# ethz-asl/okvis

Measured on NVIDIA B200. Metric: keyframe-window optimize() iters/sec (10KF/2k-lm stereo), higher is better.
Workload: dtype f64

## Files before the change

okvis_b200/csrc/okb_estimator.cu:

```cuda
#include <cuda_runtime.h>

#include <algorithm>
#include <cstddef>
#include <cstdio>
#include <cstdlib>
#include <cstring>
#include <string>
#include <thread>
#include <vector>

#include "okb_ctx.h"
#include "okb_hostpack.hpp"
#include "okb_graph.cuh"
#include "okb_kernels.cuh"
#include "okb_marg.cuh"

using namespace okb;

static std::string g_create_error;

#define OKB_CUDA(ctx, call)                                                                             \
  do {                                                                                                  \
    cudaError_t e_ = (call);                                                                            \
    if (e_ != cudaSuccess) {                                                                            \
// ... 361 lines not shown
    if (marg_n > kMaxMarg || marg_nb > kMaxMargBlocks) { c->set_error("marginalisation prior too large"); return OKB_ERR_CAPACITY; }
    int col = 0;
    for (int b = 0; b < marg_nb; ++b) {
      const int kind = D->marg->block_kind[b];
      const uint32_t idx = D->marg->block_idx[b];
      const int lim = kind == OKB_BLOCK_POSE ? K : kind == OKB_BLOCK_SPEED_BIAS ? NSB : kind == OKB_BLOCK_EXTRINSICS ? NE : -1;
      if (lim < 0) { c->set_error("marginalisation prior: unknown block kind"); return OKB_ERR_INVALID_ARG; }
      if ((int)idx >= lim) { c->set_error("marginalisation prior: block index out of range"); return OKB_ERR_INVALID_ARG; }
      if (kind != OKB_BLOCK_EXTRINSICS) col += (kind == OKB_BLOCK_SPEED_BIAS) ? 9 : 6;
      marg_xdim += (kind == OKB_BLOCK_SPEED_BIAS) ? 9 : 7;
    }
    if (col != marg_n) { c->set_error("marginalisation prior dimension mismatch"); return OKB_ERR_INVALID_ARG; }
  }
  for (int i = 0; i < D->n_pose_priors; ++i)
    if ((int)D->pose_priors[i].pose_idx >= K) { c->set_error("pose prior index out of range"); return OKB_ERR_INVALID_ARG; }
  for (int i = 0; i < D->n_sb_priors; ++i)
    if ((int)D->sb_priors[i].sb_idx >= NSB) { c->set_error("speed/bias prior index out of range"); return OKB_ERR_INVALID_ARG; }
  for (int t = 0; t < D->n_imu_terms; ++t) {
    const okb_imu_term& T = D->imu_terms[t];
    if ((int)T.pose0 >= K || (int)T.pose1 >= K || (int)T.sb0 >= NSB || (int)T.sb1 >= NSB ||
        (uint64_t)T.sample_offset + (uint64_t)T.sample_count > (uint64_t)D->n_imu_samples || T.sample_count < 2) {
      c->set_error("IMU term index out of range");
      return OKB_ERR_INVALID_ARG;
    }
  }
  for (int i = 0; i < D->n_obs; ++i) {
    const okb_observation& ob = D->obs[i];
    if ((int)ob.pose_idx >= K || (int)ob.lm_idx >= L || (int)ob.ext_idx >= NE || (int)ob.cam_idx >= NC) {
      c->set_error("observation index out of range");
      return OKB_ERR_INVALID_ARG;
    }
    if (!(ob.sqrt_info > 0.0)) { c->set_error("observation with non-positive sqrt information"); return OKB_ERR_INVALID_ARG; }
  }
  if (smemA2_bytes(K, 4 * ((6 * K + 1 + 3) / 4), 0) > (size_t)c->smem_optin) { c->set_error("window does not fit kernel A shared memory"); return OKB_ERR_CAPACITY; }

  WinStore& S = c->wins[win];
  S.uploaded = false;
  WinCaps need{K, L, D->n_obs, D->n_imu_samples, D->n_imu_terms, NE, NC, std::max(D->n_pose_priors, D->n_sb_priors), marg_n};
  need = caps_max(need, S.reserve);
  need.T = std::max(need.T, need.K);
  if (!S.arena || !caps_cover(S.caps, need)) {
    if (S.done_idx >= 0) OKB_CUDA(c, cudaEventSynchronize(c->done_ring[S.done_idx]));
    int rc = plan_arena(c, win, S.arena ? caps_max(S.caps, need) : need);
    if (rc) return rc;
  }
  S.cmd_used = 0;
  int rc = cmd_reserve(c, S, full_upload_bytes(need));
  if (rc) return rc;
  unsigned char* q;
  q = cmd_put(S, CMD_RESET_GRAPH, 0, (uint32_t)NE, (uint32_t)NC, 8 * 7 * (size_t)NE + sizeof(okb_camera) * NC);
  std::memcpy(q, D->extrinsics, 8 * 7 * (size_t)NE);
  std::memcpy(q + 8 * 7 * (size_t)NE, D->cameras, sizeof(okb_camera) * NC);
  q = cmd_put(S, CMD_SET_FRAMES, 0, (uint32_t)K, (uint32_t)NSB, 8 * (7 * (size_t)K + 9 * (size_t)NSB));
  std::memcpy(q, D->poses, 8 * 7 * (size_t)K);
  if (NSB) std::memcpy(q + 8 * 7 * (size_t)K, D->speed_bias, 8 * 9 * (size_t)NSB);
  q = cmd_put(S, CMD_SET_LANDMARKS, (uint32_t)L, 0, 1, 8 * 4 * (size_t)L);
  std::memcpy(q, D->landmarks, 8 * 4 * (size_t)L);
  if (D->n_obs) {
    q = cmd_put(S, CMD_ADD_OBS, (uint32_t)D->n_obs, 0, 0, sizeof(okb_observation) * (size_t)D->n_obs);
    std::memcpy(q, D->obs, sizeof(okb_observation) * (size_t)D->n_obs);
  }
  q = cmd_put(S, CMD_SET_IMU, 0, (uint32_t)D->n_imu_terms, (uint32_t)D->n_imu_samples,
              sizeof(okb_imu_term) * D->n_imu_terms + sizeof(okb_imu_sample) * (size_t)D->n_imu_samples);
  if (D->n_imu_terms) std::memcpy(q, D->imu_terms, sizeof(okb_imu_term) * D->n_imu_terms);
  if (D->n_imu_samples) std::memcpy(q + sizeof(okb_imu_term) * D->n_imu_terms, D->imu_samples, sizeof(okb_imu_sample) * (size_t)D->n_imu_samples);
  q = cmd_put(S, CMD_SET_POSE_PRIORS, (uint32_t)D->n_pose_priors, 0, 0, sizeof(okb_pose_prior) * D->n_pose_priors);
  if (D->n_pose_priors) std::memcpy(q, D->pose_priors, sizeof(okb_pose_prior) * D->n_pose_priors);
// ... 52 lines not shown
    std::vector<std::thread> th;
    th.reserve(T);
    for (int t = 0; t < T; ++t)
      th.emplace_back([=, &rcs]() {
        for (int i = t; i < count; i += T) {
          const int rc = upload_pack(c, first + i, descs + i);
          if (rc) { rcs[t] = rc; return; }
        }
      });
    for (auto& x : th) x.join();
  }
  for (int t = 0; t < T; ++t)
    if (rcs[t]) return rcs[t];
  return commit_range(c, first, count);
}

static int delta_begin(okb_ctx* c, int win, size_t extra, WinStore** S, WinDev** W) {
  if (!c || win < 0 || win >= c->max_windows) return OKB_ERR_INVALID_ARG;
  if (!c->wins[win].uploaded) { c->set_error("window slot not uploaded"); return OKB_ERR_INVALID_ARG; }
  cudaSetDevice(c->device);
  *S = &c->wins[win];
  *W = &c->host[win];
  return cmd_reserve(c, **S, extra + sizeof(CmdHeader) + 64);
}

extern "C" int okb_window_add_frame(okb_ctx* c, int win, const double* pose, const double* speed_bias, const okb_imu_term* term,
                                    const okb_imu_sample* samples, int n_samples) {
  WinStore* S; WinDev* W;
  if (!pose || (term && (!samples || n_samples < 2))) return OKB_ERR_INVALID_ARG;
  int rc = delta_begin(c, win, 16 * 8 + sizeof(okb_imu_term) + sizeof(okb_imu_sample) * (size_t)std::max(n_samples, 0) + sizeof(CmdHeader), &S, &W);
  if (rc) return rc;
  const int K1 = W->K + 1, NSB1 = W->NSB + (speed_bias ? 1 : 0);
  if (K1 > S->caps.K || NSB1 > S->caps.K || 6 * K1 + 9 * NSB1 > kMaxDense) { c->set_error("okb_window_add_frame: frame capacity exceeded (okb_window_reserve)"); return OKB_ERR_CAPACITY; }
  if (smemA2_bytes(K1, 4 * ((6 * K1 + 1 + 3) / 4), 0) > (size_t)c->smem_optin) { c->set_error("window does not fit kernel A shared memory"); return OKB_ERR_CAPACITY; }
  if (term) {
    if ((int)term->pose0 >= K1 || (int)term->pose1 >= K1 || (int)term->sb0 >= NSB1 || (int)term->sb1 >= NSB1 ||
        (uint64_t)term->sample_offset + term->sample_count > (uint64_t)n_samples || term->sample_count < 2) {
      c->set_error("IMU term index out of range");
      return OKB_ERR_INVALID_ARG;
    }
    if (W->n_imu + 1 > S->caps.T || W->n_samples + n_samples > S->caps.S) { c->set_error("okb_window_add_frame: IMU capacity exceeded (okb_window_reserve)"); return OKB_ERR_CAPACITY; }
  }
  if (c->shard_world > 1 && shard_box_doubles(K1, 4 * ((6 * K1 + 1 + 3) / 4)) > (size_t)c->shard_box_cap) { c->set_error("window exceeds the shard mailbox"); return OKB_ERR_CAPACITY; }
  unsigned char* q = cmd_put(*S, CMD_ADD_FRAME, 0, 0, speed_bias ? 1u : 0u, 8 * 16);
  std::memcpy(q, pose, 56);
  if (speed_bias) std::memcpy(q + 56, speed_bias, 72); else std::memset(q + 56, 0, 72);
  W->K = K1; W->NSB = NSB1;
  if (term) {
    q = cmd_put(*S, CMD_ADD_IMU_TERM, (uint32_t)n_samples, 0, 0, sizeof(okb_imu_term) + sizeof(okb_imu_sample) * (size_t)n_samples);
    std::memcpy(q, term, sizeof(okb_imu_term));
    std::memcpy(q + sizeof(okb_imu_term), samples, sizeof(okb_imu_sample) * (size_t)n_samples);
    okb_imu_term mirror = *term;
    mirror.sample_offset += (uint32_t)W->n_samples;
    S->terms.push_back(mirror);
    W->n_imu += 1; W->n_samples += n_samples;
  }
  derive_dims(*W);
  return OKB_OK;
}

extern "C" int okb_window_remove_frame(okb_ctx* c, int win, uint32_t pose_idx, uint32_t sb_idx) {
  WinStore* S; WinDev* W;
  int rc = delta_begin(c, win, 0, &S, &W);
  if (rc) return rc;
  const bool has_sb = sb_idx != 0xffffffffu;
  if ((int)pose_idx >= W->K || (has_sb && (int)sb_idx >= W->NSB) || W->K < 2) { c->set_error("okb_window_remove_frame: index out of range"); return OKB_ERR_INVALID_ARG; }
  cmd_put(*S, CMD_REMOVE_FRAME, 0, pose_idx, sb_idx, 0);
// ... 435 lines not shown

extern "C" int64_t okb_window_h2d_bytes(const okb_ctx* c, int win) {
  if (!c || win < 0 || win >= c->max_windows || !c->wins[win].uploaded) return 0;
  return (int64_t)(c->wins[win].h2d_bytes + sizeof(WinDev));
}

extern "C" int okb_window_reset(okb_ctx* c, int first, int count) {
  int rc = check_range(c, first, count);
  if (rc) return rc;
  cudaSetDevice(c->device);
  for (int i = first; i < first + count; ++i) {
    const WinStore& S = c->wins[i];
    const WinDev& W = c->host[i];
    if (W.K != S.K_init || W.NSB != S.NSB_init || W.L != S.L_init) { c->set_error("okb_window_reset: the window changed shape since its last full upload"); return OKB_ERR_INVALID_ARG; }
  }
  rc = commit_range(c, first, count);
  if (rc) return rc;
  cudaStream_t xs = c->stream_xfer;
  bool waited[okb_ctx::kDoneRing] = {};
  for (int i = first; i < first + count; ++i) {
    const WinStore& S = c->wins[i];
    if (S.done_idx >= 0 && !waited[S.done_idx]) {
      OKB_CUDA(c, cudaStreamWaitEvent(xs, c->done_ring[S.done_idx], 0));
      waited[S.done_idx] = true;
    }
  }
  k_reset<<<count, 128, 0, xs>>>(c->d_wins, first, 1);
  c->launches += 1;
  OKB_CUDA(c, cudaGetLastError());
  return OKB_OK;
}

struct RoundPlan {
  int max_chunks = 1, max_imu = 0, max_cx = 1, max_K = 1, acc_copies = 1, chol_smem = 1, solve_threads = S_THREADS, gxQ = 1, shard = 0, push_gx = 1;
  size_t smA = 0, smS = 0, smQ = 0;
};
static int plan_rounds(okb_ctx* c, int first, int count, RoundPlan& P) {
  P = RoundPlan();
  int chol_smem = 1;
  int acc_copies = 1;
  const size_t sm_two = ((size_t)c->smem_per_sm - 2048) / 2;
  for (int i = first; i < first + count; ++i)
    if (smemA2_bytes(c->host[i].K, c->host[i].dcp, 1) > std::min((size_t)c->smem_optin, sm_two) &&
        smemA2_bytes(c->host[i].K, c->host[i].dcp, 0) <= sm_two) acc_copies = 0;
  for (int i = first; i < first + count; ++i)
    if (smemA2_bytes(c->host[i].K, c->host[i].dcp, acc_copies) > (size_t)c->smem_optin) acc_copies = 0;
  int maxL = 1;
  for (int i = first; i < first + count; ++i) {
    const WinDev& W = c->host[i];
    P.max_chunks = std::max(P.max_chunks, W.n_chunks);
    P.max_imu = std::max(P.max_imu, W.n_imu);
    P.smA = std::max(P.smA, smemA2_bytes(W.K, W.dcp, acc_copies));
    P.max_cx = std::max(P.max_cx, (W.L + L1_THREADS - 1) / L1_THREADS);
    P.max_K = std::max(P.max_K, W.K);
    {
      const int wm = smemS_bytes(W.d, W.dc, W.K, W.marg_n, W.n_imu, 1) <= (size_t)c->smem_optin ? 1
                   : smemS_bytes(W.d, W.dc, W.K, W.marg_n, W.n_imu, 2) <= (size_t)c->smem_optin ? 2 : 0;
      if (wm == 0 || chol_smem == 0) chol_smem = 0;
      else if (wm == 2) chol_smem = 2;
    }
    P.smQ = std::max(P.smQ, (size_t)W.NS * sizeof(SlotCtx));
    maxL = std::max(maxL, W.L);
  }
  for (int i = first; i < first + count; ++i) {
    const WinDev& W = c->host[i];
    P.smS = std::max(P.smS, smemS_bytes(W.d, W.dc, W.K, W.marg_n, W.n_imu, chol_smem));
  }
  if (P.smS > (size_t)c->smem_optin) { c->set_error("window does not fit kernel S shared memory"); return OKB_ERR_CAPACITY; }
  if (const char* force = getenv("OKB_SOLVE_MODE")) {
    const int m = atoi(force);
    if ((m == 0 || m == 2) && chol_smem != 0 && !(chol_smem == 2 && m == 2)) {
      chol_smem = m;
      P.smS = 0;
      for (int i = first; i < first + count; ++i) {
        const WinDev& W = c->host[i];
        P.smS = std::max(P.smS, smemS_bytes(W.d, W.dc, W.K, W.marg_n, W.n_imu, chol_smem));
      }
      if (P.smS > (size_t)c->smem_optin) { c->set_error("window does not fit kernel S shared memory"); return OKB_ERR_CAPACITY; }
    }
  }
  P.acc_copies = acc_copies; P.chol_smem = chol_smem;
  P.solve_threads = (2 * count <= c->sm_count) ? 512 : S_THREADS;
  P.gxQ = std::max(1, std::min((maxL + 127) / 128, (4 * c->sm_count + count - 1) / count));
  P.shard = c->shard_world > 1 ? 1 : 0;
  P.push_gx = std::max(1, std::min(16, c->sm_count / std::max(1, count)));
  return OKB_OK;
}

static int launch_rounds(okb_ctx* c, int first, int count, const okb_solve_options& opt, int rounds, const RoundPlan& P) {
  for (int r = 0; r < rounds; ++r) {
    const dim3 gridA(P.max_chunks, count);
    static const bool imu_serial = getenv("OKB_IMU_SERIAL") != nullptr;
    if (P.max_imu > 0 && imu_serial) {
      k_imu<<<dim3((P.max_imu + 32 / IMU_G - 1) / (32 / IMU_G), count), 32, smemI_bytes(), c->stream>>>(c->d_wins, first);
      c->launches += 1;
    } else if (P.max_imu > 0) {
      cudaEventRecord(c->ev_round, c->stream);
      cudaStreamWaitEvent(c->stream_imu, c->ev_round, 0);
      k_imu<<<dim3((P.max_imu + 32 / IMU_G - 1) / (32 / IMU_G), count), 32, smemI_bytes(), c->stream_imu>>>(c->d_wins, first);
      cudaEventRecord(c->ev_imu, c->stream_imu);
      c->launches += 1;
    }
    prof_begin(c, 0);
    k_linearize<<<dim3(P.max_cx, P.max_K, count), L1_THREADS, 0, c->stream>>>(c->d_wins, first);
    k_lmblock<<<dim3(P.max_cx, count), 128, 0, c->stream>>>(c->d_wins, first);
    k_schur<<<gridA, A2_THREADS, P.smA, c->stream>>>(c->d_wins, first, P.acc_copies, opt.max_iterations);
    if (P.shard) {
      k_shard_push<<<dim3(P.push_gx, count), 256, 0, c->stream>>>(c->d_wins, first);
      c->launches += 1;
    } else if (P.max_chunks > 1) { k_reduce_partials<<<dim3(8, count), 256, 0, c->stream>>>(c->d_wins, first); c->launches += 1; }
    prof_end(c);
    c->launches += 3;
    if (P.max_imu > 0 && !imu_serial) cudaStreamWaitEvent(c->stream, c->ev_imu, 0);
    prof_begin(c, 1);
    if (P.solve_threads == 512) k_solve<512><<<count, 512, P.smS, c->stream>>>(c->d_wins, first, opt, P.chol_smem);
    else k_solve<S_THREADS><<<count, S_THREADS, P.smS, c->stream>>>(c->d_wins, first, opt, P.chol_smem);
    prof_end(c);
    c->launches += 1;
  }
  OKB_CUDA(c, cudaGetLastError());
  return OKB_OK;
}

static int launch_quality(okb_ctx* c, int first, int count, const RoundPlan& P) {
  prof_begin(c, 2);
  k_quality<<<dim3(P.gxQ, count), 128, P.smQ, c->stream>>>(c->d_wins, first);
  prof_end(c);
  c->launches += 1;
  OKB_CUDA(c, cudaGetLastError());
  return OKB_OK;
}

static int run_rounds(okb_ctx* c, int first, int count, const okb_solve_options& opt, int rounds, bool with_quality) {
  RoundPlan P;
  int rc = plan_rounds(c, first, count, P);
  if (rc) return rc;
  static const bool no_graph = getenv("OKB_NO_GRAPH") != nullptr;
  if (c->profile || no_graph || c->shard_world > 1) {
    rc = launch_rounds(c, first, count, opt, rounds, P);
// ... 488 lines not shown
```

okvis_b200/csrc/okb_kernels_lm.cuh:

```cuda
#pragma once
#include "okb_estimator.cuh"

namespace okb {

constexpr int L1_THREADS = 128;
constexpr int A2_THREADS = 192;
constexpr int A2_TILE = 32;
constexpr int kPartH = 32;

struct SlotCtx {
  SlotXf xf;
  CamIntr cam;
  int frame;
  int valid;
};
static_assert(sizeof(SlotCtx) % 8 == 0, "SlotCtx is copied as doubles");

__device__ inline void build_slot_ctx(const WinDev& W, int tid, int nthr) {
  for (int s = tid; s < W.NS; s += nthr) {
    const SlotInfo si = W.slots[s];
    SlotCtx sc;
    sc.valid = si.valid; sc.frame = s / W.CP;
    if (si.valid) { make_slot_xf(W.pose_c + 7 * si.pose_idx, W.ext + 7 * si.ext_idx, sc.xf); cam_load(W.cams[si.cam_idx], sc.cam); }
    else { for (int k = 0; k < 9; ++k) sc.xf.R[k] = 0; for (int k = 0; k < 3; ++k) sc.xf.t[k] = 0; cam_load(W.cams[0], sc.cam); }
    W.slot_ctx[s] = sc;
  }
}

__global__ void __launch_bounds__(L1_THREADS) k_linearize(const WinDev* __restrict__ wins, int win_first) {
  const WinDev& W = wins[win_first + blockIdx.z];
  const SolverState* st = W.st;
  if (st->done) return;
  const int f = blockIdx.y;
  const int cx = blockIdx.x;
  if (f >= W.K || cx * L1_THREADS >= W.L) return;
  const int tid = threadIdx.x;
  const int L = W.L, CP = W.CP;

  __shared__ SlotCtx slots[32];
// ... 162 lines not shown
  for (int c = 0; c < 3; ++c) {
    const double s2 = sc3[c] * sc3[c];
    E[c] = fmin(fmax(s2 * hd[c], kMinDiag), kMaxDiag) / s2;
  }
  const double R[6] = {H[0] + mu * E[0], H[1], H[2], H[3] + mu * E[1], H[4], H[5] + mu * E[2]};
  double Lc[6], Li[6];
  if (chol3(R, Lc)) linv3(Lc, Li);
  else {
#pragma unroll
    for (int i = 0; i < 6; ++i) Li[i] = 0.0;
    st->numeric_fail = 1;
  }
  double* Ro = W.lm_Rinv + 6 * (size_t)l;
  Ro[0] = Li[0] * Li[0] + Li[1] * Li[1] + Li[3] * Li[3];
  Ro[1] = Li[1] * Li[2] + Li[3] * Li[4];
  Ro[2] = Li[3] * Li[5];
  Ro[3] = Li[2] * Li[2] + Li[4] * Li[4];
  Ro[4] = Li[4] * Li[5];
  Ro[5] = Li[5] * Li[5];
  double* gs = W.lm_g[cur ^ 1] + 3 * (size_t)l;
  double* Es = W.lm_E[cur ^ 1] + 3 * (size_t)l;
#pragma unroll
  for (int c = 0; c < 3; ++c) { gs[c] = gl[c]; Es[c] = E[c]; }
  double* Lo = W.lm_Li + 9 * (size_t)l;
#pragma unroll
  for (int i = 0; i < 6; ++i) Lo[i] = Li[i];
  Lo[6] = Li[0] * gl[0];
  Lo[7] = Li[1] * gl[0] + Li[2] * gl[1];
  Lo[8] = Li[3] * gl[0] + Li[4] * gl[1] + Li[5] * gl[2];
}

constexpr int kLiStride = 9;

__host__ __device__ inline int schur_ldy(int dcp) { return dcp + 2; }

__host__ __device__ inline size_t schur_acc_doubles(int K) { return (size_t)(6 * K + 1) * (6 * K + 2) / 2; }
__host__ __device__ inline size_t smemA2_bytes(int K, int dcp, int acc_copies) {
  size_t b = 16;
  b += ((size_t)3 * A2_TILE * schur_ldy(dcp) + 8) * sizeof(double);
  b += (size_t)2 * K * 6 * A2_TILE * sizeof(double);
  b += (size_t)2 * A2_TILE * kLiStride * sizeof(double);
  b += (size_t)2 * A2_TILE * 4 * sizeof(double);
  b += (size_t)K * 4 * sizeof(double);
  b += (size_t)acc_copies * schur_acc_doubles(K) * sizeof(double);
  return b;
}

__device__ __forceinline__ uint32_t smem_u32(const void* p) { return (uint32_t)__cvta_generic_to_shared(p); }
__device__ __forceinline__ void mbar_init(uint64_t* bar, uint32_t count) {
  asm volatile("mbarrier.init.shared::cta.b64 [%0], %1;" ::"r"(smem_u32(bar)), "r"(count) : "memory");
}
__device__ __forceinline__ void mbar_arrive_expect_tx(uint64_t* bar, uint32_t bytes) {
  asm volatile("mbarrier.arrive.expect_tx.shared::cta.b64 _, [%0], %1;" ::"r"(smem_u32(bar)), "r"(bytes) : "memory");
}
__device__ __forceinline__ void bulk_g2s(void* dst, const void* src, uint32_t bytes, uint64_t* bar) {
  asm volatile("cp.async.bulk.shared::cluster.global.mbarrier::complete_tx::bytes [%0], [%1], %2, [%3];" ::"r"(smem_u32(dst)), "l"(src),
               "r"(bytes), "r"(smem_u32(bar))
               : "memory");
}
__device__ __forceinline__ void mbar_wait(uint64_t* bar, uint32_t parity) {
  uint32_t ok;
  do {
    asm volatile("{\n\t.reg .pred p;\n\tmbarrier.try_wait.parity.shared::cta.b64 p, [%1], %2;\n\tselp.u32 %0, 1, 0, p;\n\t}"
                 : "=r"(ok)
                 : "r"(smem_u32(bar)), "r"(parity)
                 : "memory");
  } while (!ok);
}
__device__ __forceinline__ void fence_proxy_async() { asm volatile("fence.proxy.async.shared::cta;" ::: "memory"); }

__global__ void __launch_bounds__(A2_THREADS, 2) k_schur(const WinDev* __restrict__ wins, int win_first, int acc_copies, int max_iterations) {
  const WinDev& W = wins[win_first + blockIdx.y];
  SolverState* st = W.st;
  if (st->done) return;
  if (st->iteration >= max_iterations) return;
  const int chunk = blockIdx.x;
  if (chunk >= W.n_chunks) return;
  const int tid = threadIdx.x;
  const int K = W.K, dc = W.dc, dcp = W.dcp, L = W.L;
  const int ldy = schur_ldy(dcp);

  extern __shared__ __align__(16) unsigned char smem_raw[];
  uint64_t* mbar = reinterpret_cast<uint64_t*>(smem_raw);
  double* Yt = reinterpret_cast<double*>(smem_raw + 16);
  double* sMb = Yt + (size_t)3 * A2_TILE * ldy + 8;
  double* sLib = sMb + (size_t)2 * K * 6 * A2_TILE;
  double* sXb = sLib + 2 * A2_TILE * kLiStride;
  double* tws = sXb + 2 * A2_TILE * 4;
  double* Sp = W.partA + (size_t)chunk * W.partA_stride;
  const bool acc_smem = acc_copies > 0;
  const int acc_n = (dc + 1) * (dc + 2) / 2;
  double* Sacc = acc_smem ? tws + 4 * K : Sp;
  const int n_acc = acc_smem ? acc_copies * acc_n : dcp * dcp;

  for (int f = tid; f < K; f += A2_THREADS) {
    tws[4 * f] = W.pose_c[7 * f]; tws[4 * f + 1] = W.pose_c[7 * f + 1]; tws[4 * f + 2] = W.pose_c[7 * f + 2];
  }
  for (int i = tid; i < n_acc; i += A2_THREADS) Sacc[i] = 0.0;

  const int lm_begin = chunk * W.lm_per_chunk;
  const int lm_end = min(L, lm_begin + W.lm_per_chunk);

  const int warp = tid >> 5, lane = tid & 31;
  if (tid == 0) { mbar_init(&mbar[0], 1); mbar_init(&mbar[1], 1); fence_proxy_async(); }
  __syncthreads();
  uint32_t phase_bits = 0;
  auto stage = [&](int base, int buf, uint32_t tr) {
    const int fa = tr & 0xffu, fb = tr >> 8;
    if (fa > fb || warp != A2_THREADS / 32 - 1) return;
    double* sM = sMb + (size_t)buf * K * 6 * A2_TILE;
    double* sLi = sLib + buf * A2_TILE * kLiStride;
    double* sX = sXb + buf * A2_TILE * 4;
    if (lane == 0) {
      const uint32_t m_bytes = (uint32_t)(fb - fa + 1) * 6 * A2_TILE * 8;
      mbar_arrive_expect_tx(&mbar[buf], m_bytes + A2_TILE * kLiStride * 8 + A2_TILE * 4 * 8);
      bulk_g2s(sM + (size_t)fa * 6 * A2_TILE, W.lm_M + lm_M_index(base, fa, K), m_bytes, &mbar[buf]);
      bulk_g2s(sLi, W.lm_Li + (size_t)kLiStride * base, A2_TILE * kLiStride * 8, &mbar[buf]);
      bulk_g2s(sX, W.lm_c + 4 * (size_t)base, A2_TILE * 4 * 8, &mbar[buf]);
    }
  };

  int cur_fa = -1, cur_fb = -1, lane_fmax = 0;
  int KS = 1, kg = 0, n_act = 0, n_pairs = 0, n_pass = 1;
  int a_off = 0, b_off = 0, row0 = 0, col0 = 0;
  bool on = false, aug = false;
  double acc[36];
#pragma unroll
  for (int i = 0; i < 36; ++i) acc[i] = 0.0;

  auto decode = [&](int item, int fa) {
    aug = false;
    on = item < n_act;
    if (!on) return;
    if (item < n_pairs) {
      int i = (int)((sqrtf(8.0f * (float)item + 1.0f) - 1.0f) * 0.5f);
      while (i * (i + 1) / 2 > item) --i;
      while ((i + 1) * (i + 2) / 2 <= item) ++i;
      const int j = item - i * (i + 1) / 2;
      row0 = 6 * (fa + i); col0 = 6 * (fa + j);
      lane_fmax = fa + i;
    } else {
      aug = true;
      row0 = dc; col0 = 6 * (fa + item - n_pairs);
      lane_fmax = fa + item - n_pairs;
    }
    a_off = row0; b_off = col0;
  };
  double* Ssm = tws + 4 * K;
  auto flush_smem = [&](int copy) {
    double* cp = Ssm + (size_t)copy * acc_n + col0;
    if (aug) {
      double* rp = cp + (size_t)dc * (dc + 1) / 2;
#pragma unroll
      for (int c = 0; c < 6; ++c) rp[c] += acc[c];
    } else if (row0 == col0) {
#pragma unroll
      for (int r = 0; r < 6; ++r) {
        double* rp = cp + (size_t)(row0 + r) * (row0 + r + 1) / 2;
#pragma unroll
        for (int c = 0; c <= r; ++c) rp[c] += acc[r * 6 + c];
      }
    } else {
#pragma unroll
      for (int r = 0; r < 6; ++r) {
        double* rp = cp + (size_t)(row0 + r) * (row0 + r + 1) / 2;
        double t[6];
#pragma unroll
        for (int c = 0; c < 6; ++c) t[c] = rp[c];
#pragma unroll
        for (int c = 0; c < 6; ++c) rp[c] = t[c] + acc[r * 6 + c];
      }
    }
  };
  auto flush_global = [&]() {
#pragma unroll
    for (int i = 0; i < 36; ++i) {
      const int rr = row0 + i / 6, cc = col0 + i % 6;
      if ((!aug || i < 6) && cc <= rr) Sp[(size_t)rr * dcp + cc] += acc[i];
    }
  };
  auto flush = [&]() {
    for (int o = KS >> 1; o > 0; o >>= 1) {
#pragma unroll
      for (int i = 0; i < 36; ++i) acc[i] += __shfl_down_sync(0xffffffffu, acc[i], o);
    }
    if (on && kg == 0) { if (acc_smem) flush_smem(0); else flush_global(); }
#pragma unroll
    for (int i = 0; i < 36; ++i) acc[i] = 0.0;
  };

#ifdef OKB_SCHUR_PROF
  const bool prof = (tid == 0 && chunk == 0);
  unsigned long long t_ph = 0, ph[8] = {0, 0, 0, 0, 0, 0, 0, 0};
  auto now = []() { return (unsigned long long)clock64(); };
#define SCHUR_MARK(i) do { if (prof) { const unsigned long long n_ = now(); ph[i] += n_ - t_ph; t_ph = n_; } } while (0)
  if (prof) t_ph = now();
#else
#define SCHUR_MARK(i) do { } while (0)
#endif
  int buf = 0;
  const int last_tile = (lm_end - 1) >> 5;
  uint32_t tr_cur = (lm_begin < lm_end) ? W.tile_range[lm_begin >> 5] : 1u;
  uint32_t tr_n1 = (lm_begin + A2_TILE < lm_end) ? W.tile_range[(lm_begin >> 5) + 1] : 1u;
  if (lm_begin < lm_end) stage(lm_begin, 0, tr_cur);
  for (int base = lm_begin; base < lm_end; base += A2_TILE) {
    const uint32_t tr_n2 = W.tile_range[min((base >> 5) + 2, last_tile)];
    const int nl = min(A2_TILE, lm_end - base);
    const double* sM = sMb + (size_t)buf * K * 6 * A2_TILE;
    const double* sLi = sLib + buf * A2_TILE * kLiStride;
    const double* sX = sXb + buf * A2_TILE * 4;
    if ((tr_cur & 0xffu) <= (tr_cur >> 8)) {
      mbar_wait(&mbar[buf], (phase_bits >> buf) & 1u);
      phase_bits ^= 1u << buf;
    }
    __syncthreads();
    SCHUR_MARK(0);
    if (base + A2_TILE < lm_end) stage(base + A2_TILE, buf ^ 1, tr_n1);
    SCHUR_MARK(6);
    const uint32_t tr = tr_cur;
    tr_cur = tr_n1; tr_n1 = tr_n2;
    const int fa = tr & 0xffu, fb = tr >> 8;
    buf ^= 1;
    if (fa > fb) continue;
    const int u = fb - fa + 1;
    if (fa != cur_fa || fb != cur_fb) {
      flush();
      cur_fa = fa; cur_fb = fb;
      const int um = fb - fa + 1;
      n_pairs = um * (um + 1) / 2;
      n_act = n_pairs + um;
      constexpr int NW = A2_THREADS / 32;
      const int ipw = (n_act + NW - 1) / NW;
      if (ipw <= 32) {
        n_pass = 1;
        KS = 1;
        while (2 * KS <= 8 && 2 * KS * ipw <= 32) KS *= 2;
        kg = lane % KS;
        const int il = lane / KS;
        decode(warp * ipw + il, fa);
        on = on && il < ipw;
      } else {
        n_pass = (n_act + A2_THREADS - 1) / A2_THREADS;
        KS = 1; kg = 0;
      }
    }
    SCHUR_MARK(1);
    if (tid < A2_TILE) {
      const int ll = tid;
      double* yz = Yt + (size_t)(3 * ll) * ldy + dc;
      const bool v = ll < nl;
      yz[0] = v ? sLi[ll * kLiStride + 6] : 0.0;
      yz[ldy] = v ? sLi[ll * kLiStride + 7] : 0.0;
      yz[2 * ldy] = v ? sLi[ll * kLiStride + 8] : 0.0;
    }
    for (int pidx = tid; pidx < A2_TILE * u; pidx += A2_THREADS) {
      const int ll = pidx % A2_TILE, f = fa + pidx / A2_TILE;
      double* y0 = Yt + (size_t)(3 * ll) * ldy + 6 * f;
      double* y1 = y0 + ldy;
      double* y2 = y1 + ldy;
      double M0 = 0, M1 = 0, M2 = 0, M3 = 0, M4 = 0, M5 = 0;
      if (ll < nl) {
        const double* sp = sM + (size_t)(f * 6) * A2_TILE + ll;
        M0 = sp[0]; M1 = sp[A2_TILE]; M2 = sp[2 * A2_TILE]; M3 = sp[3 * A2_TILE]; M4 = sp[4 * A2_TILE]; M5 = sp[5 * A2_TILE];
      }
      if (M0 != 0.0 || M3 != 0.0 || M5 != 0.0) {
        const double* Li = sLi + ll * kLiStride;
        const double w = sX[ll * 4 + 3];
        const double p0 = sX[ll * 4] - tws[4 * f] * w, p1 = sX[ll * 4 + 1] - tws[4 * f + 1] * w, p2 = sX[ll * 4 + 2] - tws[4 * f + 2] * w;
        const double N00 = M0 * Li[0], N01 = M0 * Li[1] + M1 * Li[2], N02 = M0 * Li[3] + M1 * Li[4] + M2 * Li[5];
        const double N10 = M1 * Li[0], N11 = M1 * Li[1] + M3 * Li[2], N12 = M1 * Li[3] + M3 * Li[4] + M4 * Li[5];
        const double N20 = M2 * Li[0], N21 = M2 * Li[1] + M4 * Li[2], N22 = M2 * Li[3] + M4 * Li[4] + M5 * Li[5];
        y0[0] = -w * N00; y0[1] = -w * N10; y0[2] = -w * N20;
        y1[0] = -w * N01; y1[1] = -w * N11; y1[2] = -w * N21;
        y2[0] = -w * N02; y2[1] = -w * N12; y2[2] = -w * N22;
        y0[3] = -(p1 * N20 - p2 * N10); y0[4] = -(p2 * N00 - p0 * N20); y0[5] = -(p0 * N10 - p1 * N00);
        y1[3] = -(p1 * N21 - p2 * N11); y1[4] = -(p2 * N01 - p0 * N21); y1[5] = -(p0 * N11 - p1 * N01);
        y2[3] = -(p1 * N22 - p2 * N12); y2[4] = -(p2 * N02 - p0 * N22); y2[5] = -(p0 * N12 - p1 * N02);
      } else {
#pragma unroll
        for (int i = 0; i < 6; ++i) { y0[i] = 0.0; y1[i] = 0.0; y2[i] = 0.0; }
      }
    }
    SCHUR_MARK(2);
    __syncthreads();
    SCHUR_MARK(3);
    const int ncols = 3 * nl;
    for (int pass = 0; pass < n_pass; ++pass) {
      if (n_pass > 1) decode(pass * A2_THREADS + tid, fa);
      if (on && lane_fmax <= fb) {
        const double* pa = Yt + a_off + (size_t)kg * ldy;
        const double* pb = Yt + b_off + (size_t)kg * ldy;
        const int step = KS * ldy;
#pragma unroll 1
        for (int k = kg; k < ncols; k += KS) {
          const double2 a01 = *reinterpret_cast<const double2*>(pa);
          const double2 a23 = *reinterpret_cast<const double2*>(pa + 2);
          const double2 a45 = *reinterpret_cast<const double2*>(pa + 4);
          const double2 b01 = *reinterpret_cast<const double2*>(pb);
          const double2 b23 = *reinterpret_cast<const double2*>(pb + 2);
          const double2 b45 = *reinterpret_cast<const double2*>(pb + 4);
          const double av[6] = {a01.x, a01.y, a23.x, a23.y, a45.x, a45.y};
          const double bv[6] = {b01.x, b01.y, b23.x, b23.y, b45.x, b45.y};
#pragma unroll
          for (int i = 0; i < 6; ++i)
#pragma unroll
            for (int j = 0; j < 6; ++j) acc[i * 6 + j] += av[i] * bv[j];
          pa += step; pb += step;
        }
      }
      if (n_pass > 1) flush();
    }
    SCHUR_MARK(4);
  }
  __syncthreads();
  if (n_pass == 1) flush();
  if (acc_smem) {
    __syncthreads();
    for (int i = tid; i < (dc + 1) * dcp; i += A2_THREADS) {
      const int r = i / dcp, cidx = i % dcp;
      if (cidx <= r) {
        const int e = r * (r + 1) / 2 + cidx;
        double v = Sacc[e];
        for (int q = 1; q < acc_copies; ++q) v += Sacc[(size_t)q * acc_n + e];
        Sp[i] = v;
      }
    }
  }
  SCHUR_MARK(5);
#ifdef OKB_SCHUR_PROF
  if (prof) for (int i = 0; i < 8; ++i) st->phase_ns[8 + i] += ph[i];
#endif
#undef SCHUR_MARK
}

__global__ void __launch_bounds__(256) k_reduce_partials(const WinDev* __restrict__ wins, int win_first) {
  const WinDev& W = wins[win_first + blockIdx.y];
  if (W.st->done || W.n_chunks <= 1) return;
  const int n = W.dcp * W.dcp;
  for (int i = blockIdx.x * blockDim.x + threadIdx.x; i < n; i += gridDim.x * blockDim.x) {
    double s = W.partA[i];
    for (int c = 1; c < W.n_chunks; ++c) s += W.partA[(size_t)c * W.partA_stride + i];
    W.partA[i] = s;
  }
}

__device__ __forceinline__ void st_release_sys_u64(unsigned long long* p, unsigned long long v) {
  asm volatile("st.release.sys.global.u64 [%0], %1;" ::"l"(p), "l"(v) : "memory");
}
__device__ __forceinline__ unsigned long long ld_acquire_sys_u64(const unsigned long long* p) {
  unsigned long long v;
  asm volatile("ld.acquire.sys.global.u64 %0, [%1];" : "=l"(v) : "l"(p) : "memory");
  return v;
}
__device__ __forceinline__ double* shard_box(const WinDev& W, int dst, int parity, int src) {
  return reinterpret_cast<double*>(W.shard_mail[dst] + kShardHeaderBytes) + ((size_t)parity * W.shard_world + src) * W.shard_box_cap;
}
__device__ __forceinline__ unsigned long long* shard_flag(const WinDev& W, int dst, size_t which, int parity, int src) {
  return reinterpret_cast<unsigned long long*>(W.shard_mail[dst] + which) + parity * kMaxShard + src;
// ... 95 lines not shown
```

Measured before the change: 196,000.

## Compute Schur complement tiles with FP64 DMMA tensor-core instructions

```diff
diff --git a/okvis_b200/csrc/okb_estimator.cu b/okvis_b200/csrc/okb_estimator.cu
--- a/okvis_b200/csrc/okb_estimator.cu
+++ b/okvis_b200/csrc/okb_estimator.cu
@@ -417,7 +417,7 @@
     }
     if (!(ob.sqrt_info > 0.0)) { c->set_error("observation with non-positive sqrt information"); return OKB_ERR_INVALID_ARG; }
   }
-  if (smemA2_bytes(K, 4 * ((6 * K + 1 + 3) / 4), 0) > (size_t)c->smem_optin) { c->set_error("window does not fit kernel A shared memory"); return OKB_ERR_CAPACITY; }
+  if (smemA2_bytes(K, 0) > (size_t)c->smem_optin) { c->set_error("window does not fit kernel A shared memory"); return OKB_ERR_CAPACITY; }
 
   WinStore& S = c->wins[win];
   S.uploaded = false;
@@ -536,7 +536,7 @@
   if (rc) return rc;
   const int K1 = W->K + 1, NSB1 = W->NSB + (speed_bias ? 1 : 0);
   if (K1 > S->caps.K || NSB1 > S->caps.K || 6 * K1 + 9 * NSB1 > kMaxDense) { c->set_error("okb_window_add_frame: frame capacity exceeded (okb_window_reserve)"); return OKB_ERR_CAPACITY; }
-  if (smemA2_bytes(K1, 4 * ((6 * K1 + 1 + 3) / 4), 0) > (size_t)c->smem_optin) { c->set_error("window does not fit kernel A shared memory"); return OKB_ERR_CAPACITY; }
+  if (smemA2_bytes(K1, 0) > (size_t)c->smem_optin) { c->set_error("window does not fit kernel A shared memory"); return OKB_ERR_CAPACITY; }
   if (term) {
     if ((int)term->pose0 >= K1 || (int)term->pose1 >= K1 || (int)term->sb0 >= NSB1 || (int)term->sb1 >= NSB1 ||
         (uint64_t)term->sample_offset + term->sample_count > (uint64_t)n_samples || term->sample_count < 2) {
@@ -1038,25 +1038,25 @@
 }
 
 struct RoundPlan {
-  int max_chunks = 1, max_imu = 0, max_cx = 1, max_K = 1, acc_copies = 1, chol_smem = 1, solve_threads = S_THREADS, gxQ = 1, shard = 0, push_gx = 1;
+  int max_chunks = 1, max_imu = 0, max_cx = 1, max_K = 1, acc_smem = 1, chol_smem = 1, solve_threads = S_THREADS, gxQ = 1, shard = 0, push_gx = 1;
   size_t smA = 0, smS = 0, smQ = 0;
 };
 static int plan_rounds(okb_ctx* c, int first, int count, RoundPlan& P) {
   P = RoundPlan();
   int chol_smem = 1;
-  int acc_copies = 1;
+  int acc_smem = 1;
   const size_t sm_two = ((size_t)c->smem_per_sm - 2048) / 2;
   for (int i = first; i < first + count; ++i)
-    if (smemA2_bytes(c->host[i].K, c->host[i].dcp, 1) > std::min((size_t)c->smem_optin, sm_two) &&
-        smemA2_bytes(c->host[i].K, c->host[i].dcp, 0) <= sm_two) acc_copies = 0;
+    if (smemA2_bytes(c->host[i].K, 1) > std::min((size_t)c->smem_optin, sm_two) &&
+        smemA2_bytes(c->host[i].K, 0) <= sm_two) acc_smem = 0;
   for (int i = first; i < first + count; ++i)
-    if (smemA2_bytes(c->host[i].K, c->host[i].dcp, acc_copies) > (size_t)c->smem_optin) acc_copies = 0;
+    if (smemA2_bytes(c->host[i].K, acc_smem) > (size_t)c->smem_optin) acc_smem = 0;
   int maxL = 1;
   for (int i = first; i < first + count; ++i) {
     const WinDev& W = c->host[i];
     P.max_chunks = std::max(P.max_chunks, W.n_chunks);
     P.max_imu = std::max(P.max_imu, W.n_imu);
-    P.smA = std::max(P.smA, smemA2_bytes(W.K, W.dcp, acc_copies));
+    P.smA = std::max(P.smA, smemA2_bytes(W.K, acc_smem));
     P.max_cx = std::max(P.max_cx, (W.L + L1_THREADS - 1) / L1_THREADS);
     P.max_K = std::max(P.max_K, W.K);
     {
@@ -1085,7 +1085,7 @@
       if (P.smS > (size_t)c->smem_optin) { c->set_error("window does not fit kernel S shared memory"); return OKB_ERR_CAPACITY; }
     }
   }
-  P.acc_copies = acc_copies; P.chol_smem = chol_smem;
+  P.acc_smem = acc_smem; P.chol_smem = chol_smem;
   P.solve_threads = (2 * count <= c->sm_count) ? 512 : S_THREADS;
   P.gxQ = std::max(1, std::min((maxL + 127) / 128, (4 * c->sm_count + count - 1) / count));
   P.shard = c->shard_world > 1 ? 1 : 0;
@@ -1110,7 +1110,7 @@
     prof_begin(c, 0);
     k_linearize<<<dim3(P.max_cx, P.max_K, count), L1_THREADS, 0, c->stream>>>(c->d_wins, first);
     k_lmblock<<<dim3(P.max_cx, count), 128, 0, c->stream>>>(c->d_wins, first);
-    k_schur<<<gridA, A2_THREADS, P.smA, c->stream>>>(c->d_wins, first, P.acc_copies, opt.max_iterations);
+    k_schur<<<gridA, A2_THREADS, P.smA, c->stream>>>(c->d_wins, first, P.acc_smem, opt.max_iterations);
     if (P.shard) {
       k_shard_push<<<dim3(P.push_gx, count), 256, 0, c->stream>>>(c->d_wins, first);
       c->launches += 1;
diff --git a/okvis_b200/csrc/okb_kernels_lm.cuh b/okvis_b200/csrc/okb_kernels_lm.cuh
--- a/okvis_b200/csrc/okb_kernels_lm.cuh
+++ b/okvis_b200/csrc/okb_kernels_lm.cuh
@@ -4,7 +4,7 @@
 namespace okb {
 
 constexpr int L1_THREADS = 128;
-constexpr int A2_THREADS = 192;
+constexpr int A2_THREADS = 256;
 constexpr int A2_TILE = 32;
 constexpr int kPartH = 32;
 
@@ -233,17 +233,17 @@
 
 constexpr int kLiStride = 9;
 
-__host__ __device__ inline int schur_ldy(int dcp) { return dcp + 2; }
+__host__ __device__ inline int schur_ldy(int K) { return 6 * K + 1 + ((3 - 6 * K) & 7); }
 
 __host__ __device__ inline size_t schur_acc_doubles(int K) { return (size_t)(6 * K + 1) * (6 * K + 2) / 2; }
-__host__ __device__ inline size_t smemA2_bytes(int K, int dcp, int acc_copies) {
+__host__ __device__ inline size_t smemA2_bytes(int K, int acc_smem) {
   size_t b = 16;
-  b += ((size_t)3 * A2_TILE * schur_ldy(dcp) + 8) * sizeof(double);
+  b += ((size_t)3 * A2_TILE * schur_ldy(K) + 8) * sizeof(double);
   b += (size_t)2 * K * 6 * A2_TILE * sizeof(double);
   b += (size_t)2 * A2_TILE * kLiStride * sizeof(double);
   b += (size_t)2 * A2_TILE * 4 * sizeof(double);
   b += (size_t)K * 4 * sizeof(double);
-  b += (size_t)acc_copies * schur_acc_doubles(K) * sizeof(double);
+  b += (size_t)acc_smem * schur_acc_doubles(K) * sizeof(double);
   return b;
 }
 
@@ -270,7 +270,11 @@
 }
 __device__ __forceinline__ void fence_proxy_async() { asm volatile("fence.proxy.async.shared::cta;" ::: "memory"); }
 
-__global__ void __launch_bounds__(A2_THREADS, 2) k_schur(const WinDev* __restrict__ wins, int win_first, int acc_copies, int max_iterations) {
+__device__ __forceinline__ void dmma_8x8x4(double& c0, double& c1, double a, double b) {
+  asm volatile("mma.sync.aligned.m8n8k4.row.col.f64.f64.f64.f64 {%0,%1}, {%2}, {%3}, {%0,%1};" : "+d"(c0), "+d"(c1) : "d"(a), "d"(b));
+}
+
+__global__ void __launch_bounds__(A2_THREADS, 2) k_schur(const WinDev* __restrict__ wins, int win_first, int acc_smem, int max_iterations) {
   const WinDev& W = wins[win_first + blockIdx.y];
   SolverState* st = W.st;
   if (st->done) return;
@@ -279,7 +283,7 @@
   if (chunk >= W.n_chunks) return;
   const int tid = threadIdx.x;
   const int K = W.K, dc = W.dc, dcp = W.dcp, L = W.L;
-  const int ldy = schur_ldy(dcp);
+  const int ldy = schur_ldy(K);
 
   extern __shared__ __align__(16) unsigned char smem_raw[];
   uint64_t* mbar = reinterpret_cast<uint64_t*>(smem_raw);
@@ -289,15 +293,14 @@
   double* sXb = sLib + 2 * A2_TILE * kLiStride;
   double* tws = sXb + 2 * A2_TILE * 4;
   double* Sp = W.partA + (size_t)chunk * W.partA_stride;
-  const bool acc_smem = acc_copies > 0;
-  const int acc_n = (dc + 1) * (dc + 2) / 2;
   double* Sacc = acc_smem ? tws + 4 * K : Sp;
-  const int n_acc = acc_smem ? acc_copies * acc_n : dcp * dcp;
+  const int n_acc = acc_smem ? (dc + 1) * (dc + 2) / 2 : dcp * dcp;
 
   for (int f = tid; f < K; f += A2_THREADS) {
     tws[4 * f] = W.pose_c[7 * f]; tws[4 * f + 1] = W.pose_c[7 * f + 1]; tws[4 * f + 2] = W.pose_c[7 * f + 2];
   }
   for (int i = tid; i < n_acc; i += A2_THREADS) Sacc[i] = 0.0;
+  if (tid < 8) Yt[(size_t)3 * A2_TILE * ldy + tid] = 0.0;
 
   const int lm_begin = chunk * W.lm_per_chunk;
   const int lm_end = min(L, lm_begin + W.lm_per_chunk);
@@ -321,73 +324,15 @@
     }
   };
 
-  int cur_fa = -1, cur_fb = -1, lane_fmax = 0;
-  int KS = 1, kg = 0, n_act = 0, n_pairs = 0, n_pass = 1;
-  int a_off = 0, b_off = 0, row0 = 0, col0 = 0;
-  bool on = false, aug = false;
-  double acc[36];
-#pragma unroll
-  for (int i = 0; i < 36; ++i) acc[i] = 0.0;
-
-  auto decode = [&](int item, int fa) {
-    aug = false;
-    on = item < n_act;
-    if (!on) return;
-    if (item < n_pairs) {
-      int i = (int)((sqrtf(8.0f * (float)item + 1.0f) - 1.0f) * 0.5f);
-      while (i * (i + 1) / 2 > item) --i;
-      while ((i + 1) * (i + 2) / 2 <= item) ++i;
-      const int j = item - i * (i + 1) / 2;
-      row0 = 6 * (fa + i); col0 = 6 * (fa + j);
-      lane_fmax = fa + i;
-    } else {
-      aug = true;
-      row0 = dc; col0 = 6 * (fa + item - n_pairs);
-      lane_fmax = fa + item - n_pairs;
-    }
-    a_off = row0; b_off = col0;
-  };
-  double* Ssm = tws + 4 * K;
-  auto flush_smem = [&](int copy) {
-    double* cp = Ssm + (size_t)copy * acc_n + col0;
-    if (aug) {
-      double* rp = cp + (size_t)dc * (dc + 1) / 2;
-#pragma unroll
-      for (int c = 0; c < 6; ++c) rp[c] += acc[c];
-    } else if (row0 == col0) {
-#pragma unroll
-      for (int r = 0; r < 6; ++r) {
-        double* rp = cp + (size_t)(row0 + r) * (row0 + r + 1) / 2;
-#pragma unroll
-        for (int c = 0; c <= r; ++c) rp[c] += acc[r * 6 + c];
-      }
-    } else {
-#pragma unroll
-      for (int r = 0; r < 6; ++r) {
-        double* rp = cp + (size_t)(row0 + r) * (row0 + r + 1) / 2;
-        double t[6];
-#pragma unroll
-        for (int c = 0; c < 6; ++c) t[c] = rp[c];
-#pragma unroll
-        for (int c = 0; c < 6; ++c) rp[c] = t[c] + acc[r * 6 + c];
-      }
-    }
-  };
-  auto flush_global = [&]() {
-#pragma unroll
-    for (int i = 0; i < 36; ++i) {
-      const int rr = row0 + i / 6, cc = col0 + i % 6;
-      if ((!aug || i < 6) && cc <= rr) Sp[(size_t)rr * dcp + cc] += acc[i];
-    }
-  };
-  auto flush = [&]() {
-    for (int o = KS >> 1; o > 0; o >>= 1) {
-#pragma unroll
-      for (int i = 0; i < 36; ++i) acc[i] += __shfl_down_sync(0xffffffffu, acc[i], o);
-    }
-    if (on && kg == 0) { if (acc_smem) flush_smem(0); else flush_global(); }
-#pragma unroll
-    for (int i = 0; i < 36; ++i) acc[i] = 0.0;
+  const int g = lane >> 2, t4 = lane & 3;
+  auto accumulate = [&](int bi, int bj, double c0, double c1, int row0, int nrow) {
+    const int i = 8 * bi + g;
+    if (i > nrow) return;
+    const int gr = i < nrow ? row0 + i : dc;
+    double* rp = Sacc + (acc_smem ? (size_t)gr * (gr + 1) / 2 : (size_t)gr * dcp) + row0;
+    const int j = 8 * bj + 2 * t4;
+    if (j <= i && j < nrow) rp[j] += c0;
+    if (j + 1 <= i && j + 1 < nrow) rp[j + 1] += c1;
   };
 
 #ifdef OKB_SCHUR_PROF
@@ -417,48 +362,25 @@
     __syncthreads();
     SCHUR_MARK(0);
     if (base + A2_TILE < lm_end) stage(base + A2_TILE, buf ^ 1, tr_n1);
-    SCHUR_MARK(6);
+    SCHUR_MARK(1);
     const uint32_t tr = tr_cur;
     tr_cur = tr_n1; tr_n1 = tr_n2;
     const int fa = tr & 0xffu, fb = tr >> 8;
     buf ^= 1;
     if (fa > fb) continue;
-    const int u = fb - fa + 1;
-    if (fa != cur_fa || fb != cur_fb) {
-      flush();
-      cur_fa = fa; cur_fb = fb;
-      const int um = fb - fa + 1;
-      n_pairs = um * (um + 1) / 2;
-      n_act = n_pairs + um;
-      constexpr int NW = A2_THREADS / 32;
-      const int ipw = (n_act + NW - 1) / NW;
-      if (ipw <= 32) {
-        n_pass = 1;
-        KS = 1;
-        while (2 * KS <= 8 && 2 * KS * ipw <= 32) KS *= 2;
-        kg = lane % KS;
-        const int il = lane / KS;
-        decode(warp * ipw + il, fa);
-        on = on && il < ipw;
-      } else {
-        n_pass = (n_act + A2_THREADS - 1) / A2_THREADS;
-        KS = 1; kg = 0;
-      }
-    }
-    SCHUR_MARK(1);
-    if (tid < A2_TILE) {
-      const int ll = tid;
-      double* yz = Yt + (size_t)(3 * ll) * ldy + dc;
-      const bool v = ll < nl;
-      yz[0] = v ? sLi[ll * kLiStride + 6] : 0.0;
-      yz[ldy] = v ? sLi[ll * kLiStride + 7] : 0.0;
-      yz[2 * ldy] = v ? sLi[ll * kLiStride + 8] : 0.0;
-    }
-    for (int pidx = tid; pidx < A2_TILE * u; pidx += A2_THREADS) {
-      const int ll = pidx % A2_TILE, f = fa + pidx / A2_TILE;
-      double* y0 = Yt + (size_t)(3 * ll) * ldy + 6 * f;
-      double* y1 = y0 + ldy;
-      double* y2 = y1 + ldy;
+    const int u = fb - fa + 1, nrow = 6 * u, row0 = 6 * fa;
+    const int T = (nrow + 8) >> 3;
+    for (int i = tid; i < 3 * A2_TILE * (min(8 * T, ldy) - nrow); i += A2_THREADS) {
+      const int k = i % (3 * A2_TILE), r = nrow + i / (3 * A2_TILE), ll = k / 3;
+      Yt[(size_t)k * ldy + r] = (r == nrow && ll < nl) ? sLi[ll * kLiStride + 6 + k % 3] : 0.0;
+    }
+    for (int p = tid; p < A2_TILE * ((u + 1) & ~1); p += A2_THREADS) {
+      const int ll = (p & 3) | ((p >> 1) & 28), fl = ((p >> 2) & 1) | ((p >> 5) & ~1);
+      if (fl >= u) continue;
+      const int f = fa + fl;
+      double2* y0 = reinterpret_cast<double2*>(Yt + (size_t)(3 * ll) * ldy + 6 * fl);
+      double2* y1 = reinterpret_cast<double2*>(Yt + (size_t)(3 * ll + 1) * ldy + 6 * fl);
+      double2* y2 = reinterpret_cast<double2*>(Yt + (size_t)(3 * ll + 2) * ldy + 6 * fl);
       double M0 = 0, M1 = 0, M2 = 0, M3 = 0, M4 = 0, M5 = 0;
       if (ll < nl) {
         const double* sp = sM + (size_t)(f * 6) * A2_TILE + ll;
@@ -471,60 +393,73 @@
         const double N00 = M0 * Li[0], N01 = M0 * Li[1] + M1 * Li[2], N02 = M0 * Li[3] + M1 * Li[4] + M2 * Li[5];
         const double N10 = M1 * Li[0], N11 = M1 * Li[1] + M3 * Li[2], N12 = M1 * Li[3] + M3 * Li[4] + M4 * Li[5];
         const double N20 = M2 * Li[0], N21 = M2 * Li[1] + M4 * Li[2], N22 = M2 * Li[3] + M4 * Li[4] + M5 * Li[5];
-        y0[0] = -w * N00; y0[1] = -w * N10; y0[2] = -w * N20;
-        y1[0] = -w * N01; y1[1] = -w * N11; y1[2] = -w * N21;
-        y2[0] = -w * N02; y2[1] = -w * N12; y2[2] = -w * N22;
-        y0[3] = -(p1 * N20 - p2 * N10); y0[4] = -(p2 * N00 - p0 * N20); y0[5] = -(p0 * N10 - p1 * N00);
-        y1[3] = -(p1 * N21 - p2 * N11); y1[4] = -(p2 * N01 - p0 * N21); y1[5] = -(p0 * N11 - p1 * N01);
-        y2[3] = -(p1 * N22 - p2 * N12); y2[4] = -(p2 * N02 - p0 * N22); y2[5] = -(p0 * N12 - p1 * N02);
+        y0[0] = make_double2(-w * N00, -w * N10); y0[1] = make_double2(-w * N20, -(p1 * N20 - p2 * N10));
+        y0[2] = make_double2(-(p2 * N00 - p0 * N20), -(p0 * N10 - p1 * N00));
+        y1[0] = make_double2(-w * N01, -w * N11); y1[1] = make_double2(-w * N21, -(p1 * N21 - p2 * N11));
+        y1[2] = make_double2(-(p2 * N01 - p0 * N21), -(p0 * N11 - p1 * N01));
+        y2[0] = make_double2(-w * N02, -w * N12); y2[1] = make_double2(-w * N22, -(p1 * N22 - p2 * N12));
+        y2[2] = make_double2(-(p2 * N02 - p0 * N22), -(p0 * N12 - p1 * N02));
       } else {
-#pragma unroll
-        for (int i = 0; i < 6; ++i) { y0[i] = 0.0; y1[i] = 0.0; y2[i] = 0.0; }
-      }
-    }
+        const double2 z = make_double2(0.0, 0.0);
+#pragma unroll
+        for (int i = 0; i < 3; ++i) { y0[i] = z; y1[i] = z; y2[i] = z; }
+      }
+    }
+    __syncthreads();
     SCHUR_MARK(2);
-    __syncthreads();
-    SCHUR_MARK(3);
-    const int ncols = 3 * nl;
-    for (int pass = 0; pass < n_pass; ++pass) {
-      if (n_pass > 1) decode(pass * A2_THREADS + tid, fa);
-      if (on && lane_fmax <= fb) {
-        const double* pa = Yt + a_off + (size_t)kg * ldy;
-        const double* pb = Yt + b_off + (size_t)kg * ldy;
-        const int step = KS * ldy;
-#pragma unroll 1
-        for (int k = kg; k < ncols; k += KS) {
-          const double2 a01 = *reinterpret_cast<const double2*>(pa);
-          const double2 a23 = *reinterpret_cast<const double2*>(pa + 2);
-          const double2 a45 = *reinterpret_cast<const double2*>(pa + 4);
-          const double2 b01 = *reinterpret_cast<const double2*>(pb);
-          const double2 b23 = *reinterpret_cast<const double2*>(pb + 2);
-          const double2 b45 = *reinterpret_cast<const double2*>(pb + 4);
-          const double av[6] = {a01.x, a01.y, a23.x, a23.y, a45.x, a45.y};
-          const double bv[6] = {b01.x, b01.y, b23.x, b23.y, b45.x, b45.y};
-#pragma unroll
-          for (int i = 0; i < 6; ++i)
-#pragma unroll
-            for (int j = 0; j < 6; ++j) acc[i * 6 + j] += av[i] * bv[j];
-          pa += step; pb += step;
+    const int ns = (3 * nl + 3) >> 2;
+    const int nb = T * (T + 1) / 2;
+    constexpr int NW = A2_THREADS / 32;
+    const int b_lo = warp * nb / NW, b_hi = (warp + 1) * nb / NW;
+    int bi = (int)((sqrtf(8.0f * (float)b_lo + 1.0f) - 1.0f) * 0.5f);
+    while (bi * (bi + 1) / 2 > b_lo) --bi;
+    while ((bi + 1) * (bi + 2) / 2 <= b_lo) ++bi;
+    int bj = b_lo - bi * (bi + 1) / 2;
+    const double* yl = Yt + (size_t)t4 * ldy + g;
+    const int kstep = 4 * ldy;
+    for (int b = b_lo; b < b_hi; b += 2) {
+      int bi1 = bi, bj1 = bj + 1;
+      if (bj1 > bi1) { ++bi1; bj1 = 0; }
+      double c00 = 0.0, c01 = 0.0, c10 = 0.0, c11 = 0.0;
+      const double* pa0 = yl + 8 * bi;
+      const double* pb0 = yl + 8 * bj;
+      const bool diag0 = bi == bj;
+      if (b + 1 < b_hi) {
+        const double* pa1 = yl + 8 * bi1;
+        const double* pb1 = yl + 8 * bj1;
+        const bool diag1 = bi1 == bj1, same_row = bi1 == bi;
+#pragma unroll 4
+        for (int s = 0; s < ns; ++s) {
+          const int o = s * kstep;
+          const double a0 = pa0[o];
+          const double b0 = diag0 ? a0 : pb0[o];
+          const double a1 = same_row ? a0 : pa1[o];
+          const double b1 = diag1 ? a1 : pb1[o];
+          dmma_8x8x4(c00, c01, a0, b0);
+          dmma_8x8x4(c10, c11, a1, b1);
         }
-      }
-      if (n_pass > 1) flush();
-    }
-    SCHUR_MARK(4);
-  }
-  __syncthreads();
-  if (n_pass == 1) flush();
+      } else {
+#pragma unroll 4
+        for (int s = 0; s < ns; ++s) {
+          const int o = s * kstep;
+          const double a0 = pa0[o];
+          const double b0 = diag0 ? a0 : pb0[o];
+          dmma_8x8x4(c00, c01, a0, b0);
+        }
+      }
+      SCHUR_MARK(3);
+      accumulate(bi, bj, c00, c01, row0, nrow);
+      if (b + 1 < b_hi) accumulate(bi1, bj1, c10, c11, row0, nrow);
+      SCHUR_MARK(4);
+      bi = bi1; bj = bj1 + 1;
+      if (bj > bi) { ++bi; bj = 0; }
+    }
+  }
   if (acc_smem) {
     __syncthreads();
     for (int i = tid; i < (dc + 1) * dcp; i += A2_THREADS) {
       const int r = i / dcp, cidx = i % dcp;
-      if (cidx <= r) {
-        const int e = r * (r + 1) / 2 + cidx;
-        double v = Sacc[e];
-        for (int q = 1; q < acc_copies; ++q) v += Sacc[(size_t)q * acc_n + e];
-        Sp[i] = v;
-      }
+      if (cidx <= r) Sp[i] = Sacc[r * (r + 1) / 2 + cidx];
     }
   }
   SCHUR_MARK(5);
```

Result: faster. 216,000 (median of 6 runs) (+10.2%).
